# lhaippp/DMHomo

Hardware: AMD Instinct MI355X
Metric: sampled images/sec (128x128, s_step=32) (higher is better)
Workload: dtype f32; 1 GPU; DGM CFG-Unet dim=64 128x128 bs=25/GPU s_step=32 cond_scale=3 (BASELINE configs[1]); global_batch=25, cfg_mode=streams, hip_graph=True, weights=seeded random init

## Files before the change

dmhomo_amd/csrc/attention.hip:

```cpp
#include "common.h"

typedef float floatx16 __attribute__((ext_vector_type(16)));

#define LA_NS 128
#define LA_PART (32 + 32 + 1024)

__global__ __launch_bounds__(256) void linattn_context_kernel(const float* __restrict__ qkv,
                                                              float* __restrict__ partial, int n, int nsplit,
                                                              const int32_t* __restrict__ rows) {
  const int jb = blockIdx.x / nsplit, sp = blockIdx.x % nsplit;
  if (rows && jb >= rows[0]) return;
  const int b = dmh_rows_phys(rows, jb);
  const int lane = threadIdx.x & 63, h = threadIdx.x >> 6;
  const int d = lane & 31, half = lane >> 5;
  const int p0 = sp * LA_NS;
  const float* base = qkv + (size_t)b * n * 384;

  float kr[LA_NS / 2], vr[LA_NS / 2];
  const float* k0 = base + (size_t)p0 * 384 + 128 + h * 32 + d;
  const float* kp = k0 + (size_t)half * 384;
#pragma unroll
  for (int i = 0; i < LA_NS / 2; ++i) {
    const int pix = p0 + 2 * i + half;
    const bool ok = pix < n;
    const float* q = ok ? kp + (size_t)i * 768 : k0;
    const float kv = q[0], vv = q[128];
    kr[i] = ok ? kv : -INFINITY;
    vr[i] = ok ? vv : 0.f;
  }
  float m = -INFINITY;
#pragma unroll
  for (int i = 0; i < LA_NS / 2; ++i) m = fmaxf(m, kr[i]);
  m = fmaxf(m, __shfl_xor(m, 32));
  float s = 0.f;
#pragma unroll
  for (int i = 0; i < LA_NS / 2; ++i) {
    kr[i] = __expf(kr[i] - m);
    s += kr[i];
  }
  s += __shfl_xor(s, 32);

  floatx16 acc;
#pragma unroll
  for (int r = 0; r < 16; ++r) acc[r] = 0.f;
#pragma unroll
  for (int i = 0; i < LA_NS / 2; ++i) acc = __builtin_amdgcn_mfma_f32_32x32x2f32(kr[i], vr[i], acc, 0, 0, 0);
  float* out = partial + ((size_t)(b * nsplit + sp) * 4 + h) * LA_PART;
  if (half == 0) {
    out[d] = m;
    out[32 + d] = s;
  }
#pragma unroll
  for (int r = 0; r < 16; ++r) {
    const int row = (r & 3) + 8 * (r >> 2) + 4 * half;
    out[64 + row * 32 + d] = acc[r];
  }
}

__global__ __launch_bounds__(1024) void linattn_merge_kernel(const float* __restrict__ partial,
                                                             float* __restrict__ ctx, int n, int nsplit,
                                                             float* __restrict__ ms, const int32_t* __restrict__ rows) {
  if (rows && (int)(blockIdx.x >> 2) >= rows[0]) return;
  const int b = dmh_rows_phys(rows, blockIdx.x >> 2), h = blockIdx.x & 3;
  const int bh = b * 4 + h;
  const int d = threadIdx.x >> 5, e = threadIdx.x & 31;
  const float* base = partial + ((size_t)b * nsplit * 4 + h) * LA_PART;
  const size_t stride = (size_t)4 * LA_PART;
  float M = -INFINITY;
#pragma unroll 8
  for (int sp = 0; sp < nsplit; ++sp) M = fmaxf(M, base[sp * stride + d]);
  float S = 0.f, acc = 0.f;
#pragma unroll 8
  for (int sp = 0; sp < nsplit; ++sp) {
    const float w = expf(base[sp * stride + d] - M);
    S = fmaf(base[sp * stride + 32 + d], w, S);
    acc = fmaf(base[sp * stride + 64 + d * 32 + e], w, acc);
  }
  ctx[(size_t)bh * 1024 + d * 32 + e] = acc / S / (float)n;
  if (ms && e == 0) {
    ms[((size_t)bh * 32 + d) * 2 + 0] = M;
    ms[((size_t)bh * 32 + d) * 2 + 1] = S;
  }
}

#define LA_TILES 4
__global__ __launch_bounds__(256) void linattn_apply_kernel(const float* __restrict__ qkv,
                                                            const float* __restrict__ ctx, float* __restrict__ out,
                                                            int n, int nblk, float scale,
                                                            const int32_t* __restrict__ rows) {
  const int jb = blockIdx.x / nblk, blk = blockIdx.x % nblk;
  if (rows && jb >= rows[0]) return;
  const int b = dmh_rows_phys(rows, jb);
  const int lane = threadIdx.x & 63, h = threadIdx.x >> 6;
  const int i = lane & 31, half = lane >> 5;
  const float* cb = ctx + ((size_t)(b * 4 + h)) * 1024;
  float bf[16];
#pragma unroll
  for (int s = 0; s < 16; ++s) bf[s] = cb[(half * 16 + s) * 32 + i];
  const float* base = qkv + (size_t)b * n * 384;
  float* ob = out + (size_t)b * n * 128;
  for (int tI = 0; tI < LA_TILES; ++tI) {
    const int p0 = (blk * LA_TILES + tI) * 32;
    if (p0 >= n) break;
    const int pix = p0 + i;
    float q[16];
    if (pix < n) {
      const float* qp = base + (size_t)pix * 384 + h * 32 + half * 16;
#pragma unroll
      for (int s4 = 0; s4 < 4; ++s4) {
        const float4 t = ld4(qp + s4 * 4);
        q[s4 * 4 + 0] = t.x;
        q[s4 * 4 + 1] = t.y;
        q[s4 * 4 + 2] = t.z;
        q[s4 * 4 + 3] = t.w;
      }
    } else {
#pragma unroll
      for (int s = 0; s < 16; ++s) q[s] = 0.f;
    }
    float m = q[0];
#pragma unroll
    for (int s = 1; s < 16; ++s) m = fmaxf(m, q[s]);
    m = fmaxf(m, __shfl_xor(m, 32));
    float sum = 0.f;
#pragma unroll
    for (int s = 0; s < 16; ++s) {
      q[s] = expf(q[s] - m);
      sum += q[s];
    }
    sum += __shfl_xor(sum, 32);
    floatx16 acc;
#pragma unroll
    for (int r = 0; r < 16; ++r) acc[r] = 0.f;
#pragma unroll
    for (int s = 0; s < 16; ++s) {
      const float a = (q[s] / sum) * scale;
      acc = __builtin_amdgcn_mfma_f32_32x32x2f32(a, bf[s], acc, 0, 0, 0);
    }
#pragma unroll
    for (int r = 0; r < 16; ++r) {
      const int row = (r & 3) + 8 * (r >> 2) + 4 * half;
      if (p0 + row < n) ob[(size_t)(p0 + row) * 128 + h * 32 + i] = acc[r];
    }
  }
}

template <bool PAG>
__global__ __launch_bounds__(256) void attention_kernel(const float* __restrict__ qkv, float* __restrict__ out, int n,
                                                        int qtiles, float scale, const int32_t* __restrict__ rows,
                                                        int pert_lo) {
  const int wid = blockIdx.x * 4 + (threadIdx.x >> 6);
  const int lane = threadIdx.x & 63;
  const int i = lane & 31, half = lane >> 5;
  const int qt = wid % qtiles;
  const int bh = wid / qtiles;
  const int h = bh & 3;
  if (rows && (bh >> 2) >= rows[0]) return;
  const int b = dmh_rows_phys(rows, bh >> 2);
  const float* base = qkv + (size_t)b * n * 384;
  const int q0 = qt * 32;
  if (PAG && b >= pert_lo) {
    const int qi = q0 + i;
    if (qi < n) {
      const float* vp = base + (size_t)qi * 384 + 256 + h * 32 + half * 16;
      float* op = out + ((size_t)b * n + qi) * 128 + h * 32 + half * 16;
#pragma unroll
      for (int s4 = 0; s4 < 4; ++s4) st4(op + s4 * 4, ld4(vp + s4 * 4));
    }
    return;
  }

  float qf[16];
  {
    const int qi = q0 + i;
    if (qi < n) {
      const float* qp = base + (size_t)qi * 384 + h * 32 + half * 16;
#pragma unroll
      for (int s4 = 0; s4 < 4; ++s4) {
        const float4 t = ld4(qp + s4 * 4);
        qf[s4 * 4 + 0] = t.x * scale;
        qf[s4 * 4 + 1] = t.y * scale;
        qf[s4 * 4 + 2] = t.z * scale;
        qf[s4 * 4 + 3] = t.w * scale;
      }
    } else {
#pragma unroll
      for (int s = 0; s < 16; ++s) qf[s] = 0.f;
    }
  }
  floatx16 oacc;
#pragma unroll
  for (int r = 0; r < 16; ++r) oacc[r] = 0.f;
  float mrun = -INFINITY, lrun = 0.f;

  for (int k0 = 0; k0 < n; k0 += 32) {
    float kf[16];
    const int ki = k0 + i;
    if (ki < n) {
      const float* kp = base + (size_t)ki * 384 + 128 + h * 32 + half * 16;
#pragma unroll
      for (int s4 = 0; s4 < 4; ++s4) {
        const float4 t = ld4(kp + s4 * 4);
        kf[s4 * 4 + 0] = t.x;
        kf[s4 * 4 + 1] = t.y;
        kf[s4 * 4 + 2] = t.z;
        kf[s4 * 4 + 3] = t.w;
      }
    } else {
#pragma unroll
      for (int s = 0; s < 16; ++s) kf[s] = 0.f;
    }
    floatx16 sacc;
#pragma unroll
    for (int r = 0; r < 16; ++r) sacc[r] = 0.f;
#pragma unroll
    for (int s = 0; s < 16; ++s) sacc = __builtin_amdgcn_mfma_f32_32x32x2f32(kf[s], qf[s], sacc, 0, 0, 0);
    float tmax = -INFINITY;
#pragma unroll
    for (int r = 0; r < 16; ++r) {
      const int key = k0 + (r & 3) + 8 * (r >> 2) + 4 * half;
      if (key >= n) sacc[r] = -INFINITY;
      tmax = fmaxf(tmax, sacc[r]);
    }
    tmax = fmaxf(tmax, __shfl_xor(tmax, 32));
    const float mnew = fmaxf(mrun, tmax);
    const float alpha = expf(mrun - mnew);
    float psum = 0.f;
#pragma unroll
    for (int r = 0; r < 16; ++r) {
      sacc[r] = expf(sacc[r] - mnew);
      psum += sacc[r];
    }
    psum += __shfl_xor(psum, 32);
    lrun = fmaf(lrun, alpha, psum);
    mrun = mnew;
#pragma unroll
    for (int r = 0; r < 16; ++r) oacc[r] *= alpha;
#pragma unroll
    for (int r = 0; r < 16; ++r) {
      const int key = k0 + (r & 3) + 8 * (r >> 2) + 4 * half;
      const float vv = (key < n) ? base[(size_t)key * 384 + 256 + h * 32 + i] : 0.f;
      oacc = __builtin_amdgcn_mfma_f32_32x32x2f32(vv, sacc[r], oacc, 0, 0, 0);
    }
  }
  const int qi = q0 + i;
  if (qi < n) {
    float* op = out + ((size_t)b * n + qi) * 128 + h * 32;
    const float inv = 1.0f / lrun;
#pragma unroll
    for (int g4 = 0; g4 < 4; ++g4) {
      float4 o;
      o.x = oacc[g4 * 4 + 0] * inv;
      o.y = oacc[g4 * 4 + 1] * inv;
      o.z = oacc[g4 * 4 + 2] * inv;
      o.w = oacc[g4 * 4 + 3] * inv;
      st4(op + 8 * g4 + 4 * half, o);
    }
  }
}

extern "C" int dmh_linattn_splits(int n) { return dmh_dims_ok({n}, 1, 1 << 26) ? cdiv(n, LA_NS) : -1; }

extern "C" int64_t dmh_linattn_partial_floats(int B, int n) {
  if (!dmh_dims_ok({B}) || !dmh_dims_ok({n}, 1, 1 << 26)) return -1;
  return (int64_t)B * dmh_linattn_splits(n) * 4 * LA_PART;
}

extern "C" int dmh_linattn_context(const float* qkv, float* partial, int B, int n, const int32_t* rows, void* stream) {
  DMH_REQUIRE(qkv && partial && B > 0 && n > 0, "dmh_linattn_context: bad arguments");
  const int ns = dmh_linattn_splits(n);
  hipLaunchKernelGGL(linattn_context_kernel, dim3(B * ns), dim3(256), 0, (hipStream_t)stream, qkv, partial, n, ns, rows);
  DMH_CHECK_LAUNCH("dmh_linattn_context");
  return DMH_OK;
}

extern "C" int dmh_linattn_merge(const float* partial, float* ctx, int B, int n, const int32_t* rows, void* stream) {
  DMH_REQUIRE(partial && ctx && B > 0 && n > 0, "dmh_linattn_merge: bad arguments");
  hipLaunchKernelGGL(linattn_merge_kernel, dim3(B * 4), dim3(1024), 0, (hipStream_t)stream, partial, ctx, n,
                     dmh_linattn_splits(n), (float*)nullptr, rows);
  DMH_CHECK_LAUNCH("dmh_linattn_merge");
  return DMH_OK;
}

extern "C" int dmh_linattn_merge_n(const float* partial, float* ctx, int B, int n, int nsplit, const int32_t* rows,
                                   void* stream) {
  DMH_REQUIRE(partial && ctx && B > 0 && n > 0 && nsplit > 0, "dmh_linattn_merge_n: bad arguments");
  hipLaunchKernelGGL(linattn_merge_kernel, dim3(B * 4), dim3(1024), 0, (hipStream_t)stream, partial, ctx, n, nsplit,
                     (float*)nullptr, rows);
  DMH_CHECK_LAUNCH("dmh_linattn_merge_n");
  return DMH_OK;
}

extern "C" int dmh_linattn_merge_ms(const float* partial, float* ctx, float* ms, int B, int n, void* stream) {
  DMH_REQUIRE(partial && ctx && ms && B > 0 && n > 0, "dmh_linattn_merge_ms: bad arguments");
  hipLaunchKernelGGL(linattn_merge_kernel, dim3(B * 4), dim3(1024), 0, (hipStream_t)stream, partial, ctx, n,
                     dmh_linattn_splits(n), ms, (const int32_t*)nullptr);
  DMH_CHECK_LAUNCH("dmh_linattn_merge_ms");
  return DMH_OK;
}

extern "C" int dmh_linattn_apply(const float* qkv, const float* ctx, float* out, int B, int n, float scale,
                                 const int32_t* rows, void* stream) {
  DMH_REQUIRE(qkv && ctx && out && B > 0 && n > 0, "dmh_linattn_apply: bad arguments");
  const int nblk = cdiv(n, 32 * LA_TILES);
  hipLaunchKernelGGL(linattn_apply_kernel, dim3(B * nblk), dim3(256), 0, (hipStream_t)stream, qkv, ctx, out, n, nblk,
                     scale, rows);
  DMH_CHECK_LAUNCH("dmh_linattn_apply");
  return DMH_OK;
}

extern "C" int dmh_attention(const float* qkv, float* out, int B, int n, float scale, const int32_t* rows, void* stream) {
  DMH_REQUIRE(qkv && out && B > 0 && n > 0, "dmh_attention: bad arguments");
  const int qtiles = cdiv(n, 32);
  const int waves = B * 4 * qtiles;
  hipLaunchKernelGGL(attention_kernel<false>, dim3(waves / 4), dim3(256), 0, (hipStream_t)stream, qkv, out, n, qtiles, scale,
                     rows, 0);
  DMH_CHECK_LAUNCH("dmh_attention");
  return DMH_OK;
}

extern "C" int dmh_attention_pag(const float* qkv, float* out, int B, int n, float scale, const int32_t* rows, int pert_lo,
                                 void* stream) {
  DMH_REQUIRE(qkv && out && B > 0 && n > 0, "dmh_attention_pag: bad arguments");
  DMH_REQUIRE(pert_lo >= 0 && pert_lo <= B, "dmh_attention_pag: pert_lo=%d outside [0, B=%d]", pert_lo, B);
  const int qtiles = cdiv(n, 32);
  const int waves = B * 4 * qtiles;
  hipLaunchKernelGGL(attention_kernel<true>, dim3(waves / 4), dim3(256), 0, (hipStream_t)stream, qkv, out, n, qtiles, scale,
                     rows, pert_lo);
  DMH_CHECK_LAUNCH("dmh_attention_pag");
  return DMH_OK;
}
```

Before: 89.42 images/s.

## Share K/V tiles across query waves via double-buffered LDS in attention

Each workgroup now handles four query tiles of the same batch/head. It cooperatively loads 64-key chunks of K and V into padded shared memory and prefetches the next chunk into registers while the current one is computed. Previously every wave streamed K and V from global memory on its own, and the V reads were strided scalar loads. The change cuts redundant global traffic and turns the V access into LDS reads. In exchange it adds barriers, LDS use that may limit occupancy, and idle waves when the query-tile count is not a multiple of four.

```diff
diff --git a/dmhomo_amd/csrc/attention.hip b/dmhomo_amd/csrc/attention.hip
--- a/dmhomo_amd/csrc/attention.hip
+++ b/dmhomo_amd/csrc/attention.hip
@@ -145,15 +145,25 @@
   }
 }
 
+#define ATT_G 4
+#define ATT_NT (64 * ATT_G)
+#define ATT_C 64
+#define ATT_P 36
+#define ATT_PASS (ATT_C * 8 / ATT_NT)
+static_assert(ATT_C % 32 == 0 && (ATT_C * 8) % ATT_NT == 0, "a chunk is whole key tiles and whole load passes");
+static_assert(2 * 2 * ATT_C * ATT_P * 4 <= 80 * 1024, "two workgroups per CU");
+
 template <bool PAG>
-__global__ __launch_bounds__(256) void attention_kernel(const float* __restrict__ qkv, float* __restrict__ out, int n,
-                                                        int qtiles, float scale, const int32_t* __restrict__ rows,
-                                                        int pert_lo) {
-  const int wid = blockIdx.x * 4 + (threadIdx.x >> 6);
+__global__ __launch_bounds__(ATT_NT) void attention_kernel(const float* __restrict__ qkv, float* __restrict__ out, int n,
+                                                           int qtiles, int ngroups, float scale,
+                                                           const int32_t* __restrict__ rows, int pert_lo) {
+  __shared__ __attribute__((aligned(16))) float ks[2][ATT_C * ATT_P];
+  __shared__ __attribute__((aligned(16))) float vs[2][ATT_C * ATT_P];
   const int lane = threadIdx.x & 63;
   const int i = lane & 31, half = lane >> 5;
-  const int qt = wid % qtiles;
-  const int bh = wid / qtiles;
+  const int bh = blockIdx.x / ngroups;
+  const int qt = (blockIdx.x % ngroups) * ATT_G + (threadIdx.x >> 6);
+  const bool live = qt < qtiles;
   const int h = bh & 3;
   if (rows && (bh >> 2) >= rows[0]) return;
   const int b = dmh_rows_phys(rows, bh >> 2);
@@ -193,55 +203,86 @@
   for (int r = 0; r < 16; ++r) oacc[r] = 0.f;
   float mrun = -INFINITY, lrun = 0.f;
 
-  for (int k0 = 0; k0 < n; k0 += 32) {
-    float kf[16];
-    const int ki = k0 + i;
-    if (ki < n) {
-      const float* kp = base + (size_t)ki * 384 + 128 + h * 32 + half * 16;
-#pragma unroll
-      for (int s4 = 0; s4 < 4; ++s4) {
-        const float4 t = ld4(kp + s4 * 4);
-        kf[s4 * 4 + 0] = t.x;
-        kf[s4 * 4 + 1] = t.y;
-        kf[s4 * 4 + 2] = t.z;
-        kf[s4 * 4 + 3] = t.w;
+  const int skey = threadIdx.x >> 3, sc4 = (threadIdx.x & 7) * 4;
+  const float* sbase = base + 128 + h * 32 + sc4;
+  float4 kreg[ATT_PASS], vreg[ATT_PASS];
+  auto fetch = [&](int c0) {
+#pragma unroll
+    for (int p = 0; p < ATT_PASS; ++p) {
+      const int key = c0 + skey + p * (ATT_NT / 8);
+      const float* g = key < n ? sbase + (size_t)key * 384 : sbase;
+      kreg[p] = ld4(g);
+      vreg[p] = ld4(g + 128);
+    }
+  };
+  auto stage = [&](int buf, int c0) {
+#pragma unroll
+    for (int p = 0; p < ATT_PASS; ++p) {
+      const int kl = skey + p * (ATT_NT / 8);
+      const bool ok = c0 + kl < n;
+      const float4 zero = make_float4(0.f, 0.f, 0.f, 0.f);
+      st4(&ks[buf][kl * ATT_P + sc4], ok ? kreg[p] : zero);
+      st4(&vs[buf][kl * ATT_P + sc4], ok ? vreg[p] : zero);
+    }
+  };
+  fetch(0);
+  stage(0, 0);
+
+  for (int c0 = 0, buf = 0; c0 < n; c0 += ATT_C, buf ^= 1) {
+    const bool more = c0 + ATT_C < n;
+    if (more) fetch(c0 + ATT_C);
+    __syncthreads();
+    if (live) {
+#pragma unroll
+      for (int kt = 0; kt < ATT_C / 32; ++kt) {
+        const int k0 = c0 + kt * 32;
+        if (k0 < n) {
+          float kf[16];
+          const float* kp = &ks[buf][(kt * 32 + i) * ATT_P + half * 16];
+#pragma unroll
+          for (int s4 = 0; s4 < 4; ++s4) {
+            const float4 t = ld4(kp + s4 * 4);
+            kf[s4 * 4 + 0] = t.x;
+            kf[s4 * 4 + 1] = t.y;
+            kf[s4 * 4 + 2] = t.z;
+            kf[s4 * 4 + 3] = t.w;
+          }
+          float vf[16];
+          const float* vp = &vs[buf][(kt * 32 + 4 * half) * ATT_P + i];
+#pragma unroll
+          for (int r = 0; r < 16; ++r) vf[r] = vp[((r & 3) + 8 * (r >> 2)) * ATT_P];
+          floatx16 sacc;
+#pragma unroll
+          for (int r = 0; r < 16; ++r) sacc[r] = 0.f;
+#pragma unroll
+          for (int s = 0; s < 16; ++s) sacc = __builtin_amdgcn_mfma_f32_32x32x2f32(kf[s], qf[s], sacc, 0, 0, 0);
+          float tmax = -INFINITY;
+#pragma unroll
+          for (int r = 0; r < 16; ++r) {
+            const int key = k0 + (r & 3) + 8 * (r >> 2) + 4 * half;
+            if (key >= n) sacc[r] = -INFINITY;
+            tmax = fmaxf(tmax, sacc[r]);
+          }
+          tmax = fmaxf(tmax, __shfl_xor(tmax, 32));
+          const float mnew = fmaxf(mrun, tmax);
+          const float alpha = expf(mrun - mnew);
+          float psum = 0.f;
+#pragma unroll
+          for (int r = 0; r < 16; ++r) {
+            sacc[r] = expf(sacc[r] - mnew);
+            psum += sacc[r];
+          }
+          psum += __shfl_xor(psum, 32);
+          lrun = fmaf(lrun, alpha, psum);
+          mrun = mnew;
+#pragma unroll
+          for (int r = 0; r < 16; ++r) oacc[r] *= alpha;
+#pragma unroll
+          for (int r = 0; r < 16; ++r) oacc = __builtin_amdgcn_mfma_f32_32x32x2f32(vf[r], sacc[r], oacc, 0, 0, 0);
+        }
       }
-    } else {
-#pragma unroll
-      for (int s = 0; s < 16; ++s) kf[s] = 0.f;
-    }
-    floatx16 sacc;
-#pragma unroll
-    for (int r = 0; r < 16; ++r) sacc[r] = 0.f;
-#pragma unroll
-    for (int s = 0; s < 16; ++s) sacc = __builtin_amdgcn_mfma_f32_32x32x2f32(kf[s], qf[s], sacc, 0, 0, 0);
-    float tmax = -INFINITY;
-#pragma unroll
-    for (int r = 0; r < 16; ++r) {
-      const int key = k0 + (r & 3) + 8 * (r >> 2) + 4 * half;
-      if (key >= n) sacc[r] = -INFINITY;
-      tmax = fmaxf(tmax, sacc[r]);
-    }
-    tmax = fmaxf(tmax, __shfl_xor(tmax, 32));
-    const float mnew = fmaxf(mrun, tmax);
-    const float alpha = expf(mrun - mnew);
-    float psum = 0.f;
-#pragma unroll
-    for (int r = 0; r < 16; ++r) {
-      sacc[r] = expf(sacc[r] - mnew);
-      psum += sacc[r];
-    }
-    psum += __shfl_xor(psum, 32);
-    lrun = fmaf(lrun, alpha, psum);
-    mrun = mnew;
-#pragma unroll
-    for (int r = 0; r < 16; ++r) oacc[r] *= alpha;
-#pragma unroll
-    for (int r = 0; r < 16; ++r) {
-      const int key = k0 + (r & 3) + 8 * (r >> 2) + 4 * half;
-      const float vv = (key < n) ? base[(size_t)key * 384 + 256 + h * 32 + i] : 0.f;
-      oacc = __builtin_amdgcn_mfma_f32_32x32x2f32(vv, sacc[r], oacc, 0, 0, 0);
-    }
+    }
+    if (more) stage(buf ^ 1, c0 + ATT_C);
   }
   const int qi = q0 + i;
   if (qi < n) {
@@ -312,9 +353,9 @@
 extern "C" int dmh_attention(const float* qkv, float* out, int B, int n, float scale, const int32_t* rows, void* stream) {
   DMH_REQUIRE(qkv && out && B > 0 && n > 0, "dmh_attention: bad arguments");
   const int qtiles = cdiv(n, 32);
-  const int waves = B * 4 * qtiles;
-  hipLaunchKernelGGL(attention_kernel<false>, dim3(waves / 4), dim3(256), 0, (hipStream_t)stream, qkv, out, n, qtiles, scale,
-                     rows, 0);
+  const int ngroups = cdiv(qtiles, ATT_G);
+  hipLaunchKernelGGL(attention_kernel<false>, dim3(B * 4 * ngroups), dim3(ATT_NT), 0, (hipStream_t)stream, qkv, out, n, qtiles,
+                     ngroups, scale, rows, 0);
   DMH_CHECK_LAUNCH("dmh_attention");
   return DMH_OK;
 }
@@ -324,9 +365,9 @@
   DMH_REQUIRE(qkv && out && B > 0 && n > 0, "dmh_attention_pag: bad arguments");
   DMH_REQUIRE(pert_lo >= 0 && pert_lo <= B, "dmh_attention_pag: pert_lo=%d outside [0, B=%d]", pert_lo, B);
   const int qtiles = cdiv(n, 32);
-  const int waves = B * 4 * qtiles;
-  hipLaunchKernelGGL(attention_kernel<true>, dim3(waves / 4), dim3(256), 0, (hipStream_t)stream, qkv, out, n, qtiles, scale,
-                     rows, pert_lo);
+  const int ngroups = cdiv(qtiles, ATT_G);
+  hipLaunchKernelGGL(attention_kernel<true>, dim3(B * 4 * ngroups), dim3(ATT_NT), 0, (hipStream_t)stream, qkv, out, n, qtiles,
+                     ngroups, scale, rows, pert_lo);
   DMH_CHECK_LAUNCH("dmh_attention_pag");
   return DMH_OK;
 }
```

Measured after the change: 90.00 images/s (median of 6 runs). No clear change (+0.6%).
